# mohammadmarghzari/monte-carlo-portfolio

Hardware: AMD Instinct MI355X
Metric: simulated paths/sec (16 assets x 252 steps) + VaR abs-err vs NumPy ref (higher is better)
Workload: dtype f32; 1 GPU; configs[1]: 16 synthetic assets, 1,000,000 paths per GPU, 252 steps, fp32, full pass = paths + moments + exact VaR/CVaR; n_assets=16, n_steps=252, parallelism=path-sharded x1, math=exact

## Files before the change

### monte_carlo_portfolio_amd/csrc/mcp_api.cpp

```cpp
#include <hip/hip_runtime.h>
#include <dlfcn.h>

#include <algorithm>
#include <cmath>
#include <cstdarg>
#include <cstdio>
#include <cstdlib>
#include <cstring>
#include <mutex>
#include <new>
#include <string>
#include <vector>

#include "../../include/mcport.h"
#include "mcp_device.h"
#include "mcp_paths.h"
#include "mcp_stats_kernels.h"

#ifndef MCP_EXP_LEAN
#define MCP_EXP_LEAN 1
#endif

namespace {

thread_local std::string g_err;

int fail(int code, const char* fmt, ...) {
  char buf[512];
  va_list ap;
  va_start(ap, fmt);
  vsnprintf(buf, sizeof buf, fmt, ap);
  va_end(ap);
  g_err = buf;
  return code;
}

#define HIP_TRY(expr)                                                                       \
  do {                                                                                      \
    hipError_t e_ = (expr);                                                                 \
    if (e_ != hipSuccess) return fail(MCP_E_HIP, "%s: %s", #expr, hipGetErrorString(e_)); \
  } while (0)

constexpr int KT_WIDE = 8;
constexpr int K_PAD = 512;
using mcp::SWEEP_MIN_K;

int env_sweep_mt() {
  static const int v = [] { const char* e = getenv("MCP_SWEEP_MT"); return e ? atoi(e) : 0; }();
  return v;
}
bool uses_sweep(int K) { return K >= SWEEP_MIN_K && env_sweep_mt() >= 0; }
// ... 992 lines not shown
                              (unsigned long long*)ln.d_hist, ln.stream));
  fill_hz(s.hz, rq, ln);
  s.mdd = rq.dd ? ln.d_mdd : nullptr;
  s.mdd_stride = rq.dd ? ln.mdd_stride : 0;
  s.bt = boot_block(rq, ln);
  s.st = student_block(rq);
  if (rq.garch) s.gv = garch_block(rq.gv, N);
  if (rq.cash) s.cf.flows = ln.d_flows;
  if (rq.overlay) s.ov = overlay_block(rq, ln, N);
  if (rq.rebalanced) { s.period = rq.reb->period; s.cost = (float)rq.reb->cost; }
  if (rq.src == SRC_FHS) s.fh = filt_block(rq, ln, N);
  mcp::PathKernel k = {};
  k.logc = prm->compounding == MCP_COMPOUND_LOG;
  k.fh = rq.src == SRC_FHS;
  k.boot = rq.src == SRC_BOOT || k.fh;
  k.blds = k.fh ? mcp::filt_fits_lds((uint64_t)rq.filt->n_rows, nb) : k.boot && mcp::boot_fits_lds((uint64_t)rq.boot->n_rows, nb);
  k.stt = rq.src == SRC_T;
  if (ln.attr) {
    static const mcp_garch none = {0.0, 0.0, 1.0, 0};
    k.family = mcp::FAM_AT;
    k.stt = k.gv = true;
    a.partials = nullptr;
    a.hist = nullptr;
    if (!rq.garch) s.gv = garch_block(&none, N);
    s.at = attr_block(ln, N);
  } else {
    k.family = rq.overlay ? mcp::FAM_OV : rq.cash ? mcp::FAM_CF : rq.rebalanced ? mcp::FAM_REB : rq.dd ? mcp::FAM_DD : rq.hz ? mcp::FAM_HZ : mcp::FAM_PLAIN;
    k.dd = rq.overlay && rq.dd;
    k.gv = rq.garch;
    k.kt8 = K > 1;
    k.native = (prm->flags & MCP_FLAG_NATIVE_MATH) != 0;
    k.fold = (prm->flags & MCP_FLAG_FOLD) != 0;
    k.uhi = MCP_EXP_LEAN && plain && !rq.anti && !k.kt8 && !k.native && !k.fold && nb <= mcp::LEAN_MAX_NB && mcp::lean_range(a.path_begin, a.n_paths);
    if (rq.anti) {
      static const mcp_garch none = {0.0, 0.0, 1.0, 0};
      k.anti = true;
      if (k.stt || k.gv) {
        k.stt = k.gv = true;
        if (!rq.garch) s.gv = garch_block(&none, N);
      }
    }
  }
  const hipError_t e = k_launch[nb - 1](k, s, ln.stream);
  if (e != hipSuccess) return fail(MCP_E_HIP, "path kernel launch (family %d): %s", k.family, hipGetErrorString(e));
  return MCP_OK;
}

static Launch make_launch(const float* d_packed, const double* d_pivot, uint64_t seed, uint64_t path_begin, uint64_t n_paths,
                          float* d_terminal, uint64_t stride, void* d_partials, void* d_hist, void* stream) {
  Launch ln;
  ln.d_packed = d_packed;
  ln.d_pivot = d_pivot;
  ln.seed = seed;
  ln.path_begin = path_begin;
  ln.n_paths = n_paths;
  ln.d_terminal = d_terminal;
  ln.stride = stride;
  ln.d_partials = d_partials;
  ln.d_hist = d_hist;
  ln.stream = (hipStream_t)stream;
  return ln;
}

static int launch_checked(const mcp_params* prm, const Request& rq, const Launch& ln) {
  if (int rc = check_request(prm, rq, ln.n_paths, &ln)) return rc;
  return launch_paths_impl(prm, rq, ln);
// ... 1109 lines not shown
```

### monte_carlo_portfolio_amd/csrc/mcp_paths.h

```cpp
#pragma once
#include <hip/hip_runtime.h>
#include <stdint.h>

#include <type_traits>

#include "../../include/mcport.h"
#include "mcp_device.h"
#include "mcp_stats_kernels.h"

#ifndef MCP_MIN_WAVES
#define MCP_MIN_WAVES 6
#endif
#ifndef MCP_MIN_WAVES_BIG
#define MCP_MIN_WAVES_BIG 1
#endif
#ifndef MCP_MIN_WAVES_REB
#define MCP_MIN_WAVES_REB 5
#endif
#ifndef MCP_MIN_WAVES_REB8
#define MCP_MIN_WAVES_REB8 4
#endif
#ifndef MCP_MIN_WAVES_CF8
#define MCP_MIN_WAVES_CF8 5
#endif
#ifndef MCP_MIN_WAVES_OV
#define MCP_MIN_WAVES_OV 4
#endif
#ifndef MCP_MIN_WAVES_OV8
#define MCP_MIN_WAVES_OV8 4
#endif
#ifndef MCP_MIN_WAVES_AT
#define MCP_MIN_WAVES_AT 5
#endif
#ifndef MCP_MIN_WAVES_ANTI
#define MCP_MIN_WAVES_ANTI 5
#endif
#ifndef MCP_EXP_VKEYS
#define MCP_EXP_VKEYS 1
#endif
#ifndef MCP_EXP_BOOT_SWIZZLE
#define MCP_EXP_BOOT_SWIZZLE 1
#endif
#ifndef MCP_EXP_LDSPAR
#define MCP_EXP_LDSPAR 1
#endif

namespace mcp {

typedef float f32x2 __attribute__((ext_vector_type(2)));

#ifdef MCP_DIAG_CLOCK
extern __device__ unsigned long long mcp_diag_stamps[2 * 8192];
#endif

template <class A>
__device__ __forceinline__ const __attribute__((address_space(4))) A* kernarg() {
  typedef const __attribute__((address_space(4))) A* cst_p;
  cst_p k = (cst_p)__builtin_amdgcn_kernarg_segment_ptr();
  asm volatile("" : "+s"(k));
  return k;
}
#define MCP_HAS_MEMBER(m)                                                 \
  template <class A, class = void> struct has_##m : std::false_type {}; \
  template <class A> struct has_##m<A, std::void_t<decltype(A::m)>> : std::true_type {};
MCP_HAS_MEMBER(hz) MCP_HAS_MEMBER(mdd) MCP_HAS_MEMBER(bt) MCP_HAS_MEMBER(st) MCP_HAS_MEMBER(gv) MCP_HAS_MEMBER(cf)
MCP_HAS_MEMBER(ov) MCP_HAS_MEMBER(at) MCP_HAS_MEMBER(period) MCP_HAS_MEMBER(pr)
MCP_HAS_MEMBER(fh) MCP_HAS_MEMBER(p_hi)
#undef MCP_HAS_MEMBER

struct PathArgs {
  const float* __restrict__ packed;
  float* __restrict__ terminal;
  const float4* __restrict__ tables;
  const double* __restrict__ pivot;
  MomentPartial* __restrict__ partials;
  unsigned long long* __restrict__ hist;
  uint64_t slots;
  double v0d;
  double inv_v0d;
  int32_t v0_pow2;
  uint64_t seed, path_begin, n_paths, stride;
  int32_t n_steps, n_portfolios, k_begin, compounding;
  int32_t k_count;
  float v0;
  uint32_t fold_offset;
};

struct PathArgsLean : PathArgs {
  uint32_t p_hi;
  uint32_t pad;
};
template <class A>
__device__ __forceinline__ uint32_t uniform_hi(const A& a) {
  if constexpr (has_p_hi<A>::value) return a.p_hi;
  else return 0u;
}

struct PathArgsDD : PathArgs {
  float* __restrict__ mdd;
  uint64_t mdd_stride;
};

struct PathArgsHZ : PathArgs {
  float* __restrict__ hz;
  uint64_t hz_stride;
  int32_t n_horizons;
  int32_t steps[MCP_MAX_HORIZONS];
};

struct BootArgs {
  const float4* __restrict__ rows;
  uint64_t thr;
  uint32_t n_rows;
  uint32_t pad;
};
struct PathArgsBT : PathArgs { BootArgs bt; };
struct PathArgsBTHZ : PathArgsHZ { BootArgs bt; };
template <class A>
__device__ __forceinline__ BootArgs boot_args(const A& a) {
  if constexpr (has_bt<A>::value) return a.bt;
  else return BootArgs{};
}
struct PathArgsRB : PathArgsHZ {
  BootArgs bt;
  int32_t period;
  float cost;
};
struct StudentArgs {
// ... 127 lines not shown
}

struct PathLaunchArgs {
  PathArgsHZ hz;
  float* mdd;
  uint64_t mdd_stride;
  BootArgs bt;
  StudentArgs st;
  GarchArgs gv;
  CashArgs cf;
  OverlayArgs ov;
  AttrArgs at;
  int32_t period;
  float cost;
  PairArgs pr;
  FiltArgs fh;
};
template <class A>
inline A make_args(const PathLaunchArgs& s) {
  A x;
  if constexpr (has_hz<A>::value) static_cast<PathArgsHZ&>(x) = s.hz;
  else static_cast<PathArgs&>(x) = s.hz;
  if constexpr (has_mdd<A>::value) { x.mdd = s.mdd; x.mdd_stride = s.mdd_stride; }
  if constexpr (has_bt<A>::value) x.bt = s.bt;
  if constexpr (has_st<A>::value) x.st = s.st;
  if constexpr (has_gv<A>::value) x.gv = s.gv;
  if constexpr (has_cf<A>::value) x.cf = s.cf;
  if constexpr (has_ov<A>::value) x.ov = s.ov;
  if constexpr (has_at<A>::value) x.at = s.at;
  if constexpr (has_period<A>::value) { x.period = s.period; x.cost = s.cost; }
  if constexpr (has_pr<A>::value) x.pr = s.pr;
  if constexpr (has_fh<A>::value) x.fh = s.fh;
  if constexpr (has_p_hi<A>::value) { x.p_hi = (uint32_t)(s.hz.path_begin >> 32); x.pad = 0u; }
  return x;
}

__host__ __device__ constexpr bool boot_fits_lds(uint64_t n_rows, int nb) { return n_rows * (uint64_t)nb <= (uint64_t)ICDF_LDS_ENTRIES; }
__host__ __device__ constexpr bool filt_fits_lds(uint64_t n_rows, int nb) {
  return n_rows * (uint64_t)nb + (n_rows + 3) / 4 <= (uint64_t)ICDF_LDS_ENTRIES;
}
template <int NB>
struct BootSwizzle {
  static constexpr int G = (NB & -NB) > 16 ? 16 : (NB & -NB);
  static constexpr int SHIFT = G == 16 ? 0 : G == 8 ? 1 : G == 4 ? 2 : G == 2 ? 3 : 4;
  static constexpr uint32_t MASK = (uint32_t)G - 1u;
  __device__ static __forceinline__ uint32_t of(uint32_t j) { return MCP_EXP_BOOT_SWIZZLE ? (j >> SHIFT) & MASK : 0u; }
};

__device__ __forceinline__ double wave_sum(double v) {
#pragma unroll
  for (int o = 32; o > 0; o >>= 1) v += __shfl_xor(v, o, 64);
  return v;
}
__device__ __forceinline__ double wave_min(double v) {
#pragma unroll
  for (int o = 32; o > 0; o >>= 1) v = fmin(v, __shfl_xor(v, o, 64));
  return v;
}
__device__ __forceinline__ double wave_max(double v) {
#pragma unroll
  for (int o = 32; o > 0; o >>= 1) v = fmax(v, __shfl_xor(v, o, 64));
  return v;
}

__device__ __forceinline__ float wave_minf(float v) {
#pragma unroll
  for (int o = 32; o > 0; o >>= 1) v = fminf(v, __shfl_xor(v, o, 64));
  return v;
}
__device__ __forceinline__ float wave_maxf(float v) {
#pragma unroll
  for (int o = 32; o > 0; o >>= 1) v = fmaxf(v, __shfl_xor(v, o, 64));
  return v;
}

__device__ __forceinline__ void lds_hist_add(uint32_t* h, uint32_t digit, bool active) {
  unsigned long long todo = __ballot(active);
  const int lane = threadIdx.x & 63;
#pragma unroll 1
  for (int it = 0; it < 4 && todo; it++) {
    const int leader = __ffsll((long long)todo) - 1;
    const uint32_t d0 = (uint32_t)__builtin_amdgcn_readlane((int)digit, leader);
    const bool same = active && digit == d0;
    const unsigned long long m = __ballot(same);
    if (lane == leader) atomicAdd(&h[d0], (uint32_t)__popcll(m));
    todo &= ~m;
    active = active && !same;
  }
  if (active) atomicAdd(&h[digit], 1u);
}

__device__ __forceinline__ double terminal_to_x(float term, double v0, int compounding) {
  return compounding == MCP_COMPOUND_LOG ? expm1((double)term) : (double)term / v0 - 1.0;
}

constexpr int PATH_BLOCK = 256;

struct PathFlagsOff {
  static constexpr bool NATIVE = false, FOLD = false, LOGC = false, DD = false, HZ = false, BOOT = false, BLDS = false, REB = false,
                        STT = false, CF = false, OV = false, GV = false, AT = false, ANTI = false, FH = false, UHI = false;
};

enum BoundsKind { BK_PATHS, BK_REB, BK_CF, BK_OV, BK_AT, BK_ANTI };
constexpr int min_waves(BoundsKind kind, int NB, int KT, int PPT) {
  if (kind == BK_ANTI) return (NB <= 4 && PPT == 1 && KT == 1) ? MCP_MIN_WAVES_ANTI : 1;
  if (NB <= 4 && PPT == 1 && KT == 1)
    return kind == BK_REB ? MCP_MIN_WAVES_REB : kind == BK_OV ? MCP_MIN_WAVES_OV : kind == BK_AT ? MCP_MIN_WAVES_AT : MCP_MIN_WAVES;
  if (NB <= 4 && PPT == 1 && kind != BK_PATHS && kind != BK_AT)
    return kind == BK_REB ? MCP_MIN_WAVES_REB8 : kind == BK_CF ? MCP_MIN_WAVES_CF8 : MCP_MIN_WAVES_OV8;
  return (KT == 1 && PPT == 1) ? MCP_MIN_WAVES_BIG : 1;
}
#define MCP_BOUNDS(kind) __launch_bounds__(PATH_BLOCK, min_waves(kind, NB, KT, PPT))

template <int NB, int KT, int PPT, bool NATIVE_, bool FOLD_ = false, bool LOGC_ = false>
__global__ void MCP_BOUNDS(BK_PATHS) mc_paths_kernel(const PathArgs a) {
  struct F : PathFlagsOff { enum : bool { NATIVE = NATIVE_, FOLD = FOLD_, LOGC = LOGC_ }; };
#include "mcp_paths_body.inc"
}

template <int NB, bool LOGC_>
__global__ void __launch_bounds__(PATH_BLOCK, min_waves(BK_PATHS, NB, 1, 1)) mc_paths_lean_kernel(const PathArgsLean a) {
  constexpr int KT = 1, PPT = 1;
  struct F : PathFlagsOff { enum : bool { LOGC = LOGC_, UHI = true }; };
#include "mcp_paths_body.inc"
}

template <int NB, int KT, int PPT, bool LOGC_>
__global__ void MCP_BOUNDS(BK_PATHS) mc_paths_dd_kernel(const PathArgsDD a) {
  struct F : PathFlagsOff { enum : bool { DD = true, LOGC = LOGC_ }; };
#include "mcp_paths_body.inc"
}

template <int NB, int KT, int PPT, bool LOGC_>
__global__ void MCP_BOUNDS(BK_PATHS) mc_paths_hz_kernel(const PathArgsHZ a) {
  struct F : PathFlagsOff { enum : bool { HZ = true, LOGC = LOGC_ }; };
#include "mcp_paths_body.inc"
}

template <int NB, int KT, int PPT, bool LOGC_, bool BLDS_>
__global__ void MCP_BOUNDS(BK_PATHS) mc_paths_boot_kernel(const PathArgsBT a) {
  struct F : PathFlagsOff { enum : bool { BOOT = true, LOGC = LOGC_, BLDS = BLDS_ }; };
#include "mcp_paths_body.inc"
}

template <int NB, int KT, int PPT, bool LOGC_, bool BLDS_>
__global__ void MCP_BOUNDS(BK_PATHS) mc_paths_boot_hz_kernel(const PathArgsBTHZ a) {
  struct F : PathFlagsOff { enum : bool { HZ = true, BOOT = true, LOGC = LOGC_, BLDS = BLDS_ }; };
#include "mcp_paths_body.inc"
}
template <int NB, int KT, int PPT, bool BOOT_, bool BLDS_>
__global__ void MCP_BOUNDS(BK_REB) mc_paths_reb_kernel(const PathArgsRB a) {
  struct F : PathFlagsOff { enum : bool { REB = true, BOOT = BOOT_, BLDS = BLDS_ }; };
#include "mcp_paths_body.inc"
}

template <int NB, int KT, int PPT>
__global__ void MCP_BOUNDS(BK_PATHS) mc_paths_t_kernel(const PathArgsT a) {
  struct F : PathFlagsOff { enum : bool { STT = true }; };
#include "mcp_paths_body.inc"
// ... 65 lines not shown
```

### monte_carlo_portfolio_amd/csrc/mcp_paths_body.inc

```
  constexpr bool NATIVE = F::NATIVE, FOLD = F::FOLD, LOGC = F::LOGC, DD = F::DD, HZ = F::HZ, BOOT = F::BOOT, BLDS = F::BLDS, REB = F::REB,
                 STT = F::STT, CF = F::CF, OV = F::OV, GV = F::GV, AT = F::AT, ANTI = F::ANTI, FH = F::FH, UHI = F::UHI;
  static_assert(!UHI || (KT == 1 && PPT == 1 && !(NATIVE || FOLD || DD || HZ || BOOT || REB || STT || CF || OV || GV || AT || ANTI || FH)),
                "uniform high counter word: the plain Gaussian walk of one portfolio only");
  static_assert(!FH || (BOOT && HZ && !(LOGC || REB || CF || STT || GV || OV || AT || DD)), "filtered rows: the bootstrap's segmented walk only");
  constexpr int N4 = 4 * NB;
  constexpr int EM = ANTI ? 2 * PPT : PPT;
  static_assert(!ANTI || !(NATIVE || FOLD || BOOT || REB || CF || OV || AT || FH), "antithetic pairs: the lean Gaussian and GARCH walks only");
  typedef const __attribute__((address_space(4))) float* cfloat_p;
  cfloat_p mu = (cfloat_p)a.packed;
  cfloat_p Lp = mu + N4;
  cfloat_p Wk = mu + N4 + N4 * (N4 / 2 + 1) + (size_t)a.k_begin * N4;
  const int kt = min(KT, a.n_portfolios - a.k_begin);
  __shared__ float4 s_tab[ICDF_LDS_ENTRIES];
  if constexpr (!NATIVE && !BOOT) {
    for (int i = threadIdx.x; i < ICDF_ENTRIES; i += PATH_BLOCK) s_tab[ICDF_PAD + i] = a.tables[i];
  }
  BootArgs bt{};
  if constexpr (BOOT) bt = boot_args(a);
  if constexpr (BOOT && BLDS) {
    for (uint32_t i = threadIdx.x; i < bt.n_rows * (uint32_t)NB; i += PATH_BLOCK) {
      const uint32_t j = i / NB, q = i % NB;
      s_tab[j * NB + (q ^ BootSwizzle<NB>::of(j))] = bt.rows[i];
    }
  }
  const float* fshock = nullptr;
  if constexpr (FH) fshock = filt_args(a)->shock;
  if constexpr (FH && BLDS) {
    for (uint32_t i = threadIdx.x; i < (bt.n_rows + 3u) / 4u; i += PATH_BLOCK) s_tab[bt.n_rows * (uint32_t)NB + i] = ((const float4*)fshock)[i];
  }
  constexpr bool LDS_MU = MCP_EXP_LDSPAR >= 1 && !NATIVE && !FOLD && !BOOT;
  constexpr bool LDS_W = MCP_EXP_LDSPAR >= 2 && !NATIVE && !FOLD && !BOOT && KT == 1;
  float* const s_par0 = (float*)&s_tab[0];
  if constexpr (LDS_MU) {
    if (threadIdx.x < N4) { s_par0[threadIdx.x] = mu[threadIdx.x]; if (LDS_W) s_par0[N4 + threadIdx.x] = Wk[threadIdx.x]; }
// ... 11 lines not shown
  }
  if (threadIdx.x < PATH_BLOCK / 64) s_cnt[threadIdx.x] = 0ull;
  if constexpr (AT) {
    double* const s_at = attr_wave_slots<N4>();
    for (int i = threadIdx.x; i < (PATH_BLOCK / 64) * attr_record_len(N4); i += PATH_BLOCK) s_at[i] = 0.0;
  }
  if constexpr (ANTI) {
    if (threadIdx.x < (PATH_BLOCK / 64) * KT) pair_wave_slots<KT>()[threadIdx.x] = 0.0;
  }
  __syncthreads();
  const IcdfConsts kc = icdf_consts<UHI>();
  PhiloxKeys ks = philox_keys((uint32_t)a.seed, (uint32_t)(a.seed >> 32));
#if MCP_EXP_VKEYS
#pragma unroll
  for (int r = 0; r < 10; r++) { asm volatile("" : "+v"(ks.k0[r])); asm volatile("" : "+v"(ks.k1[r])); }
#endif
  typedef const __attribute__((address_space(3))) float* lfloat_p;
  PhiloxUniformKeys sk{};
  uint32_t uhi = 0u;
  lfloat_p par_lds = nullptr;
  if constexpr (UHI) {
    sk = philox_uniform_keys((uint32_t)a.seed, (uint32_t)(a.seed >> 32));
    uhi = uniform_hi(a);
    par_lds = (lfloat_p)s_par0;
  }
  const int T = a.n_steps;
  constexpr bool logc = LOGC;

  const uint64_t tile = (uint64_t)PATH_BLOCK * PPT;
  const uint64_t n_tiles = (a.n_paths + tile - 1) / tile;
#ifdef MCP_DIAG_CLOCK
  const unsigned long long diag_t0 = __builtin_amdgcn_s_memtime(), diag_r0 = __builtin_amdgcn_s_memrealtime();
#endif
  for (uint64_t tl = blockIdx.x; tl < n_tiles; tl += gridDim.x) {
    uint64_t p[PPT];
    bool live[PPT];
    uint32_t plo[PPT], phi[PPT];
    float V[EM][KT];
    float Pk[EM][KT], Qk[EM][KT];
    uint32_t jrow[PPT];
    f32x2 Bs[PPT][N4 / 2];
    float Ps[PPT][N4];
    float gh[PPT];
    f32x2 At[PPT][N4 / 2];
#pragma unroll
    for (int e = 0; e < PPT; e++) {
      p[e] = tl * tile + (uint64_t)e * PATH_BLOCK + threadIdx.x;
      live[e] = p[e] < a.n_paths;
      const uint64_t g = a.path_begin + p[e];
      plo[e] = (uint32_t)g; phi[e] = (uint32_t)(g >> 32);
#pragma unroll
      for (int k = 0; k < KT; k++) V[e][k] = logc ? 0.0f : a.v0;
      if constexpr (BOOT) jrow[e] = 0u;
      if constexpr (GV) gh[e] = garch_args(a)->h0;
      if constexpr (FH) gh[e] = filt_args(a)->h0;
      if constexpr (REB) {
#pragma unroll
        for (int m = 0; m < N4 / 2; m++) Bs[e][m] = f32x2{0.0f, 0.0f};
      }
      if constexpr (AT) {
#pragma unroll
        for (int m = 0; m < N4 / 2; m++) At[e][m] = f32x2{0.0f, 0.0f};
      }
      if constexpr (DD) {
#pragma unroll
        for (int k = 0; k < KT; k++) { Pk[e][k] = -__builtin_inff(); Qk[e][k] = logc ? 0.0f : 1.0f; }
      }
      if constexpr (OV) {
        typedef const __attribute__((address_space(4))) float* cspot_p;
        const cspot_p sp = (cspot_p)kernarg<PathArgsOV>()->ov.spot;
#pragma unroll
        for (int i = 0; i < N4; i++) Ps[e][i] = sp[i];
      }
      if constexpr (ANTI) {
#pragma unroll
        for (int k = 0; k < KT; k++) {
          V[PPT + e][k] = V[e][k];
          if constexpr (DD) { Pk[PPT + e][k] = Pk[e][k]; Qk[PPT + e][k] = Qk[e][k]; }
        }
      }
    }

    if constexpr (REB) {
      int nd;
      {
// ... 68 lines not shown
          for (int e = 0; e < PPT; e++)
#pragma unroll
            for (int m = 0; m < N4 / 2; m++) Bs[e][m] = f32x2{0.0f, 0.0f};
          const int per = cs->period;
          nd = per < T - t ? t + per : T;
        }
      }
    } else if constexpr (HZ) {
      typedef const __attribute__((address_space(4))) PathArgsHZ* chz_p;
      chz_p hk = (chz_p)__builtin_amdgcn_kernarg_segment_ptr();
      const int n_seg = hk->n_horizons + 1;
      int t = 0;
      for (int seg = 0; seg < n_seg; seg++) {
        const int t_end = seg < n_seg - 1 ? hk->steps[seg] : T;
        for (; t < t_end; t++) {
#include "mcp_paths_step.inc"
        }
        if (seg < n_seg - 1) {
          const auto hs = kernarg<PathArgsHZ>();
          float* const row = hs->hz + (size_t)(seg * a.n_portfolios + a.k_begin) * hs->hz_stride;
#pragma unroll
          for (int e = 0; e < PPT; e++)
            if (live[e]) {
#pragma unroll
              for (int k = 0; k < KT; k++)
                if (k < kt) {
                  if constexpr (ANTI) *(float2*)&row[(size_t)k * hs->hz_stride + 2 * p[e]] = make_float2(V[e][k], V[PPT + e][k]);
                  else row[(size_t)k * hs->hz_stride + p[e]] = V[e][k];
                }
            }
        }
      }
    } else {
      for (int t = 0; t < T; t++) {
#include "mcp_paths_step.inc"
      }
    }

    if constexpr (AT) {
      const auto ak = &kernarg<PathArgsAT>()->at;
      asm volatile("" : "+s"(kargs));
      const double e_c = kargs->pivot[a.k_begin], e_var = ak->var[a.k_begin], e_v0d = kargs->v0d;
      int tid = threadIdx.x;
      asm volatile("" : "+v"(tid));
      const int lane = tid & 63, wv = tid >> 6;
      double* const slot = attr_wave_slots<N4>() + wv * attr_record_len(N4);
      double dv[PPT];
      bool tail[PPT];
      double cn = 0.0, ct = 0.0, s1 = 0.0;
#pragma unroll
      for (int e = 0; e < PPT; e++) {
        const double x = terminal_to_x(V[e][0], e_v0d, MCP_COMPOUND_SIMPLE);
        tail[e] = live[e] && x <= e_var;
        dv[e] = live[e] ? x - e_c : 0.0;
        cn += live[e] ? 1.0 : 0.0;
        ct += tail[e] ? 1.0 : 0.0;
        s1 += dv[e];
      }
      cn = wave_sum(cn); ct = wave_sum(ct); s1 = wave_sum(s1);
      if (lane == 0) { slot[0] += cn; slot[1] += ct; slot[2] += s1; }
#pragma unroll
      for (int i = 0; i < N4; i++) {
        double sa = 0.0, st = 0.0, sx = 0.0;
#pragma unroll
        for (int e = 0; e < PPT; e++) {
          const double ai = live[e] ? (double)((i & 1) ? At[e][i / 2].y : At[e][i / 2].x) : 0.0;
          sa += ai;
// ... 14 lines not shown
            for (int e = 0; e < PPT; e++)
              if (live[e]) cb[((size_t)a.k_begin * n_live + i) * cs + p[e]] = (i & 1) ? At[e][i / 2].y : At[e][i / 2].x;
          }
      }
    } else {
#pragma unroll
    for (int e = 0; e < PPT; e++) {
      if (live[e]) {
#pragma unroll
        for (int k = 0; k < KT; k++)
          if (k < kt) {
            if constexpr (ANTI) *(float2*)&a.terminal[(size_t)(a.k_begin + k) * a.stride + 2 * p[e]] = make_float2(V[e][k], V[PPT + e][k]);
            else a.terminal[(size_t)(a.k_begin + k) * a.stride + p[e]] = V[e][k];
          }
        if constexpr (DD && OV) {
          const auto dk = kernarg<PathArgsOV>();
#pragma unroll
          for (int k = 0; k < KT; k++)
            if (k < kt) dk->mdd[(size_t)(a.k_begin + k) * dk->mdd_stride + p[e]] = Qk[e][k];
        } else if constexpr (DD) {
          const auto dk = kernarg<PathArgsDD>();
#pragma unroll
          for (int k = 0; k < KT; k++)
            if (k < kt) {
              if constexpr (ANTI) *(float2*)&dk->mdd[(size_t)(a.k_begin + k) * dk->mdd_stride + 2 * p[e]] = make_float2(Qk[e][k], Qk[PPT + e][k]);
              else dk->mdd[(size_t)(a.k_begin + k) * dk->mdd_stride + p[e]] = Qk[e][k];
            }
        }
      }
    }
    }

    asm volatile("" : "+s"(kargs));
    if (kargs->partials != nullptr) {
      const double* __restrict__ e_pivot = kargs->pivot;
      unsigned long long* __restrict__ e_hist = kargs->hist;
      const double e_v0d = kargs->v0d;
      int tid = threadIdx.x;
      asm volatile("" : "+v"(tid));
      const int lane = tid & 63, wv = tid >> 6;
      unsigned long long cnt = 0;
#pragma unroll
      for (int e = 0; e < PPT; e++) cnt += (unsigned long long)((EM / PPT) * __popcll(__ballot(live[e])));
      if (lane == 0) s_cnt[wv] += cnt;
#pragma unroll 1
      for (int k = 0; k < kt; k++) {
        const double c = e_pivot ? e_pivot[a.k_begin + k] : 0.0;
        double d1 = 0.0, d2 = 0.0;
        float mn = __builtin_inff(), mx = -__builtin_inff();
        double dm[EM];
#pragma unroll
        for (int e = 0; e < EM; e++) {
          float v = V[e][0];
#pragma unroll
          for (int kk = 1; kk < KT; kk++) v = (kk == k) ? V[e][kk] : v;
          if constexpr (ANTI) dm[e] = 0.0;
          if (live[e % PPT]) {
            const double d = terminal_to_x(v, e_v0d, logc ? MCP_COMPOUND_LOG : MCP_COMPOUND_SIMPLE) - c;
            d1 += d;
            d2 = __builtin_fma(d, d, d2);
            mn = fminf(mn, v);
            mx = fmaxf(mx, v);
            if constexpr (ANTI) dm[e] = d;
          }
          if (e_hist) lds_hist_add(s_hist, float_to_key(v) >> 21, live[e % PPT]);
        }
        d1 = wave_sum(d1); d2 = wave_sum(d2); mn = wave_minf(mn); mx = wave_maxf(mx);
        if (lane == 0) {
          s_mom[wv][k][0] += d1; s_mom[wv][k][1] += d2;
          s_ext[wv][k][0] = fminf(s_ext[wv][k][0], mn); s_ext[wv][k][1] = fmaxf(s_ext[wv][k][1], mx);
        }
        if constexpr (ANTI) {
          double cr = 0.0;
#pragma unroll
          for (int e = 0; e < PPT; e++) cr = __builtin_fma(dm[e], dm[PPT + e], cr);
          cr = wave_sum(cr);
          if (lane == 0) pair_wave_slots<KT>()[wv * KT + k] += cr;
        }
        if (e_hist) {
          __syncthreads();
          unsigned long long* out = e_hist + (size_t)(a.k_begin + k) * 2 * MCP_SELECT_BINS;
          for (int i = tid; i < MCP_SELECT_BINS; i += PATH_BLOCK) {
            const uint32_t h = s_hist[i];
            if (h) { atomicAdd(&out[i], (unsigned long long)h); s_hist[i] = 0u; }
          }
          __syncthreads();
        }
      }
    }
  }

#ifdef MCP_DIAG_CLOCK
  if (threadIdx.x == 0 && blockIdx.x < 8192) {
    mcp_diag_stamps[2 * blockIdx.x] = __builtin_amdgcn_s_memtime() - diag_t0;
    mcp_diag_stamps[2 * blockIdx.x + 1] = __builtin_amdgcn_s_memrealtime() - diag_r0;
  }
#endif
  asm volatile("" : "+s"(kargs));
  if (kargs->partials != nullptr) {
    __syncthreads();
    if ((int)threadIdx.x < kt) {
      const int k = threadIdx.x;
      MomentPartial o;
      o.s1 = (s_mom[0][k][0] + s_mom[1][k][0]) + (s_mom[2][k][0] + s_mom[3][k][0]);
      o.s2 = (s_mom[0][k][1] + s_mom[1][k][1]) + (s_mom[2][k][1] + s_mom[3][k][1]);
      o.vmin = fminf(fminf(s_ext[0][k][0], s_ext[1][k][0]), fminf(s_ext[2][k][0], s_ext[3][k][0]));
      o.vmax = fmaxf(fmaxf(s_ext[0][k][1], s_ext[1][k][1]), fmaxf(s_ext[2][k][1], s_ext[3][k][1]));
      o.n = (s_cnt[0] + s_cnt[1]) + (s_cnt[2] + s_cnt[3]);
      kargs->partials[(size_t)(a.k_begin + k) * kargs->slots + blockIdx.x] = o;
      if constexpr (ANTI) {
        const double* const s_cr = pair_wave_slots<KT>();
        pair_cross(a)[(size_t)(a.k_begin + k) * gridDim.x + blockIdx.x] = (s_cr[k] + s_cr[KT + k]) + (s_cr[2 * KT + k] + s_cr[3 * KT + k]);
      }
    }
  }
  if constexpr (AT) {
    __syncthreads();
    const auto ak = &kernarg<PathArgsAT>()->at;
    const double* const s_at = attr_wave_slots<N4>();
    constexpr int RL = attr_record_len(N4);
    if ((int)threadIdx.x < RL) {
      const int j = threadIdx.x;
      ak->partials[((size_t)a.k_begin * gridDim.x + blockIdx.x) * RL + j] = (s_at[j] + s_at[RL + j]) + (s_at[2 * RL + j] + s_at[3 * RL + j]);
    }
  }
```

### monte_carlo_portfolio_amd/csrc/mcp_paths_inst.hip

```cpp
#include <cstdlib>

#include "mcp_paths.h"
#include "mcp_stats_kernels.h"

#ifndef MCP_NB
#error "compile with -DMCP_NB=<1..16>"
#endif

#define MCP_CAT_(a, b) a##b
#define MCP_CAT(a, b) MCP_CAT_(a, b)

namespace mcp {

static size_t lds_pad() {
  static const size_t pad = [] { const char* e = getenv("MCP_PATHS_LDS_PAD"); return e ? (size_t)atol(e) : (size_t)0; }();
  return pad;
}

template <int KT, class A>
static hipError_t run(void (*kernel)(A), const PathLaunchArgs& s, hipStream_t stream) {
  A x = make_args<A>(s);
  const int grid = path_grid(x.n_paths);
  for (x.k_begin = 0; x.k_begin < x.n_portfolios; x.k_begin += KT) {
    kernel<<<grid, PATH_BLOCK, lds_pad(), stream>>>(x);
    const hipError_t e = hipGetLastError();
    if (e != hipSuccess) return e;
  }
  return hipSuccess;
}
#define MCP_ROW(cond, ...) \
  if (cond) return run<KT>(__VA_ARGS__, s, stream)

template <int KT>
static hipError_t ladder(const PathKernel& k, const PathLaunchArgs& s, hipStream_t stream) {
  constexpr int NB = MCP_NB;
  const bool lg = k.logc;
  const bool gauss = !k.boot && !k.stt && !k.gv;
  const bool t = k.stt && !k.gv && !k.boot, g = k.gv && !k.boot;
  const bool bl = k.boot && k.blds && !k.stt && !k.gv && !k.fh, bg = k.boot && !k.blds && !k.stt && !k.gv && !k.fh;
  if (k.fh) {
    const bool ok = (k.family == FAM_PLAIN || k.family == FAM_HZ) && k.boot && !k.stt && !k.gv && !k.native && !k.anti && !lg;
    MCP_ROW(ok && k.blds, mc_paths_fhs_kernel<NB, KT, 1, true>);
    MCP_ROW(ok && !k.blds, mc_paths_fhs_kernel<NB, KT, 1, false>);
    return hipErrorInvalidValue;
  }
  if (k.anti) {
    const bool lean = gauss && !k.native, gw = k.stt && k.gv && !k.boot && !k.native && !lg;
    switch (k.family) {
      case FAM_PLAIN:
        MCP_ROW(lean && lg, mc_paths_anti_kernel<NB, KT, 1, true, PathArgsA>);
        MCP_ROW(lean && !lg, mc_paths_anti_kernel<NB, KT, 1, false, PathArgsA>);
        MCP_ROW(gw, mc_paths_anti_kernel<NB, KT, 1, false, PathArgsGA>);
        break;
      case FAM_DD:
        MCP_ROW(lean && lg, mc_paths_anti_kernel<NB, KT, 1, true, PathArgsADD>);
        MCP_ROW(lean && !lg, mc_paths_anti_kernel<NB, KT, 1, false, PathArgsADD>);
        MCP_ROW(gw, mc_paths_anti_kernel<NB, KT, 1, false, PathArgsGADD>);
        break;
      case FAM_HZ:
// ... 40 lines not shown
      MCP_ROW(gauss && !lg, mc_paths_reb_kernel<NB, KT, 1, false, false>);
      MCP_ROW(bl && !lg, mc_paths_reb_kernel<NB, KT, 1, true, true>);
      MCP_ROW(bg && !lg, mc_paths_reb_kernel<NB, KT, 1, true, false>);
      break;
    case FAM_CF:
      MCP_ROW(gauss && !lg, mc_paths_cf_kernel<NB, KT, 1, false, false, false>);
      MCP_ROW(t && !lg, mc_paths_cf_kernel<NB, KT, 1, false, false, true>);
      MCP_ROW(bl && !lg, mc_paths_cf_kernel<NB, KT, 1, true, true, false>);
      MCP_ROW(bg && !lg, mc_paths_cf_kernel<NB, KT, 1, true, false, false>);
      break;
    case FAM_OV:
      MCP_ROW(gauss && !lg && !k.dd, mc_paths_ov_kernel<NB, KT, 1, false, false>);
      MCP_ROW(gauss && !lg && k.dd, mc_paths_ov_kernel<NB, KT, 1, false, true>);
      MCP_ROW(t && !lg && !k.dd, mc_paths_ov_kernel<NB, KT, 1, true, false>);
      MCP_ROW(t && !lg && k.dd, mc_paths_ov_kernel<NB, KT, 1, true, true>);
      break;
  }
  return hipErrorInvalidValue;
}

hipError_t MCP_CAT(launch_paths_nb, MCP_NB)(const PathKernel& k, const PathLaunchArgs& s, hipStream_t stream) {
  constexpr int NB = MCP_NB, KT = 1;
  if (k.anti && (k.fold || k.family == FAM_AT)) return hipErrorInvalidValue;
  if (k.fh && (k.fold || k.family == FAM_AT)) return hipErrorInvalidValue;
  if (k.fold) {
    const bool ok = k.family == FAM_PLAIN && !k.boot && !k.stt && !k.gv && !k.native && !k.kt8;
    MCP_ROW(ok && k.logc, mc_paths_kernel<NB, 1, 1, false, true, true>);
    MCP_ROW(ok && !k.logc, mc_paths_kernel<NB, 1, 1, false, true, false>);
    return hipErrorInvalidValue;
  }
  if (k.uhi) {
    if constexpr (NB <= LEAN_MAX_NB) {
      const bool ok = k.family == FAM_PLAIN && !k.boot && !k.stt && !k.gv && !k.native && !k.kt8 && !k.anti && !k.fh;
      MCP_ROW(ok && k.logc, mc_paths_lean_kernel<NB, true>);
      MCP_ROW(ok && !k.logc, mc_paths_lean_kernel<NB, false>);
    }
    return hipErrorInvalidValue;
  }
  if (k.family == FAM_AT) {
    MCP_ROW(!k.kt8 && !k.native && !k.logc && !k.boot, mc_paths_attr_kernel<NB, 1, 1>);
    return hipErrorInvalidValue;
  }
  return k.kt8 ? ladder<8>(k, s, stream) : ladder<1>(k, s, stream);
}
#undef MCP_ROW

}
```

### monte_carlo_portfolio_amd/csrc/mcp_route.h

```cpp
#pragma once
#include <stdint.h>

namespace mcp {

inline bool lean_range(uint64_t path_begin, uint64_t n_paths) {
  if (n_paths == 0) return false;
  const uint64_t last = path_begin + (n_paths - 1);
  return last >= path_begin && (path_begin >> 32) == (last >> 32);
}

}
```

### monte_carlo_portfolio_amd/csrc/mcp_stats_kernels.h

```cpp
#pragma once
#include <hip/hip_runtime.h>
#include <stdint.h>

#include "../../include/mcport.h"
#include "mcp_route.h"

namespace mcp {

struct SelectState {
  uint32_t prefix;
  uint32_t pad;
  uint64_t rank;
};

struct Quantile {
  double x_lo, x_hi, var;
  double level2;
  uint64_t n_tail;
  uint64_t pad;
};

struct MomentPartial {
  double s1, s2;
  float vmin, vmax;
  unsigned long long n;
};
static_assert(sizeof(MomentPartial) == 32, "MomentPartial is 32 bytes");

constexpr int PATH_GRID_CAP = 8192;
constexpr int SWEEP_MIN_K = 17;
constexpr int SWEEP_TILE_PATHS = 64;

__host__ __device__ inline int path_grid(uint64_t n) {
  uint64_t tiles = (n + 255) / 256;
  if (tiles < 1) tiles = 1;
  return (int)(tiles < (uint64_t)PATH_GRID_CAP ? tiles : (uint64_t)PATH_GRID_CAP);
}
__host__ __device__ inline uint64_t moment_slots(bool sweep, uint64_t n) {
  return sweep ? (n + SWEEP_TILE_PATHS - 1) / SWEEP_TILE_PATHS + (n == 0) : (uint64_t)path_grid(n);
}

__host__ __device__ inline int stream_slots(int K) {
  const int s = 16384 / (K < 1 ? 1 : K);
  return s > 2048 ? 2048 : (s < 1 ? 1 : s);
}

struct PathArgs;
struct PathLaunchArgs;

constexpr int LEAN_MAX_NB = 4;
enum PathFamily { FAM_PLAIN, FAM_DD, FAM_HZ, FAM_REB, FAM_CF, FAM_OV, FAM_AT };
struct PathKernel {
  int family;
  bool logc, boot, blds, stt, dd, gv, kt8, native, fold, anti, fh, uhi;
};

typedef hipError_t (*launch_paths_fn)(const PathKernel& k, const PathLaunchArgs& args, hipStream_t stream);
#define MCP_DECL_NB(n) hipError_t launch_paths_nb##n(const PathKernel& k, const PathLaunchArgs& args, hipStream_t stream);
MCP_DECL_NB(1) MCP_DECL_NB(2) MCP_DECL_NB(3) MCP_DECL_NB(4) MCP_DECL_NB(5) MCP_DECL_NB(6) MCP_DECL_NB(7) MCP_DECL_NB(8)
MCP_DECL_NB(9) MCP_DECL_NB(10) MCP_DECL_NB(11) MCP_DECL_NB(12) MCP_DECL_NB(13) MCP_DECL_NB(14) MCP_DECL_NB(15) MCP_DECL_NB(16)
#undef MCP_DECL_NB

hipError_t launch_sweep_shared(int nb, int mt, bool native, const PathArgs& args, hipStream_t stream);
hipError_t launch_sweep_shared_p0(int nb, int mt, bool native, const PathArgs& args, hipStream_t stream);
hipError_t launch_sweep_shared_p1(int nb, int mt, bool native, const PathArgs& args, hipStream_t stream);
hipError_t launch_sweep_shared_p2(int nb, int mt, bool native, const PathArgs& args, hipStream_t stream);
hipError_t launch_sweep_shared_p3(int nb, int mt, bool native, const PathArgs& args, hipStream_t stream);
hipError_t launch_sweep_paths(int nb, int mt, bool native, const PathArgs& args, hipStream_t stream);
hipError_t launch_normals(const uint32_t* x, uint64_t n, const float4* table, float* z, hipStream_t s);

hipError_t launch_pass0(const mcp_params& prm, int K, const float* terminal, uint64_t stride, uint64_t n, const double* pivot,
                        uint64_t slots, MomentPartial* partials, unsigned long long* hist, hipStream_t s);
hipError_t launch_scan(const mcp_params& prm, int K, int pass, uint64_t n, uint64_t rank_lo, uint64_t rank_hi, uint64_t slots,
                       const MomentPartial* partials, const double* below, const double* pivot, unsigned long long* hist,
                       SelectState* state, mcp_record* record, hipStream_t s);
hipError_t launch_hist(const mcp_params& prm, int K, int pass, const float* terminal, uint64_t stride, uint64_t n,
                       const SelectState* state, const double* pivot, double* below, unsigned long long* hist, hipStream_t s);
hipError_t launch_final(const mcp_params& prm, int K, uint64_t n, double gamma, uint64_t rank_lo, uint64_t rank_hi,
                        const double* below, unsigned long long* hist, const SelectState* state, mcp_record* record,
                        Quantile* quant, mcp_stats* stats_or_null, hipStream_t s);
hipError_t launch_stats(const mcp_params& prm, int K, int world, const mcp_record* gathered, const Quantile* quant,
                        mcp_stats* out, hipStream_t s);
hipError_t launch_zero(void* p, size_t bytes, hipStream_t s);
hipError_t launch_count_rows(const float* values, uint64_t stride, uint64_t n, int rows, bool has_target, float target,
                             unsigned long long* counts, hipStream_t s);
hipError_t launch_sum_u64(unsigned long long* const* bufs, int nsrc, size_t words, hipStream_t s);
hipError_t launch_attr_merge(const double* partials, int K, int blocks, int len, double* out, hipStream_t s);
// ... 7 lines not shown
```

Before: 447.9 million paths/s.

## Split lean path walk into time segments to fill tail waves

Adds a segmented variant of the lean path kernel. Each launch covers a whole number of resident-block waves of (tile, time-segment) units, and the path value is carried between segments through the terminal buffer. A host-side cost model picks the segment count from occupancy and the tile count, to cut the idle tail of the last partial wave. The trade is extra launches, a global read and write of path state at each segment boundary, and a reliance on the RNG being addressable by step so the walk can resume mid-path.

```diff
diff --git a/monte_carlo_portfolio_amd/csrc/mcp_api.cpp b/monte_carlo_portfolio_amd/csrc/mcp_api.cpp
--- a/monte_carlo_portfolio_amd/csrc/mcp_api.cpp
+++ b/monte_carlo_portfolio_amd/csrc/mcp_api.cpp
@@ -17,6 +17,9 @@
 #include "mcp_paths.h"
 #include "mcp_stats_kernels.h"
 
+#ifndef MCP_EXP_SEGMENTS
+#define MCP_EXP_SEGMENTS 1
+#endif
 #ifndef MCP_EXP_LEAN
 #define MCP_EXP_LEAN 1
 #endif
@@ -1075,6 +1078,13 @@
     k.native = (prm->flags & MCP_FLAG_NATIVE_MATH) != 0;
     k.fold = (prm->flags & MCP_FLAG_FOLD) != 0;
     k.uhi = MCP_EXP_LEAN && plain && !rq.anti && !k.kt8 && !k.native && !k.fold && nb <= mcp::LEAN_MAX_NB && mcp::lean_range(a.path_begin, a.n_paths);
+    if (k.uhi) {
+      const char* const ks = getenv("MCP_TIME_SEGMENTS");
+      const char* const cs = getenv("MCP_SEGMENT_CAP");
+      const long kf = ks ? atol(ks) : 0, cf = cs ? atol(cs) : 0;
+      k.seg_forced = !MCP_EXP_SEGMENTS ? 1 : kf < 0 ? 0 : kf > prm->n_steps ? prm->n_steps : (int32_t)kf;
+      k.seg_cap = cf > 0 && cf <= (long)mcp::SEG_GRID_CAP ? (uint32_t)cf : 0u;
+    }
     if (rq.anti) {
       static const mcp_garch none = {0.0, 0.0, 1.0, 0};
       k.anti = true;
diff --git a/monte_carlo_portfolio_amd/csrc/mcp_paths.h b/monte_carlo_portfolio_amd/csrc/mcp_paths.h
--- a/monte_carlo_portfolio_amd/csrc/mcp_paths.h
+++ b/monte_carlo_portfolio_amd/csrc/mcp_paths.h
@@ -6,6 +6,7 @@
 
 #include "../../include/mcport.h"
 #include "mcp_device.h"
+#include "mcp_route.h"
 #include "mcp_stats_kernels.h"
 
 #ifndef MCP_MIN_WAVES
@@ -65,7 +66,7 @@
   template <class A> struct has_##m<A, std::void_t<decltype(A::m)>> : std::true_type {};
 MCP_HAS_MEMBER(hz) MCP_HAS_MEMBER(mdd) MCP_HAS_MEMBER(bt) MCP_HAS_MEMBER(st) MCP_HAS_MEMBER(gv) MCP_HAS_MEMBER(cf)
 MCP_HAS_MEMBER(ov) MCP_HAS_MEMBER(at) MCP_HAS_MEMBER(period) MCP_HAS_MEMBER(pr)
-MCP_HAS_MEMBER(fh) MCP_HAS_MEMBER(p_hi)
+MCP_HAS_MEMBER(fh) MCP_HAS_MEMBER(p_hi) MCP_HAS_MEMBER(first_unit)
 #undef MCP_HAS_MEMBER
 
 struct PathArgs {
@@ -94,6 +95,21 @@
 __device__ __forceinline__ uint32_t uniform_hi(const A& a) {
   if constexpr (has_p_hi<A>::value) return a.p_hi;
   else return 0u;
+}
+
+struct PathArgsSeg : PathArgsLean {
+  uint32_t first_unit;
+  int32_t n_seg;
+};
+template <class A>
+__device__ __forceinline__ uint32_t seg_first_unit(const A& a) {
+  if constexpr (has_first_unit<A>::value) return a.first_unit;
+  else return 0u;
+}
+template <class A>
+__device__ __forceinline__ int32_t seg_count(const A& a) {
+  if constexpr (has_first_unit<A>::value) return a.n_seg;
+  else return 1;
 }
 
 struct PathArgsDD : PathArgs {
@@ -287,6 +303,7 @@
   if constexpr (has_pr<A>::value) x.pr = s.pr;
   if constexpr (has_fh<A>::value) x.fh = s.fh;
   if constexpr (has_p_hi<A>::value) { x.p_hi = (uint32_t)(s.hz.path_begin >> 32); x.pad = 0u; }
+  if constexpr (has_first_unit<A>::value) { x.first_unit = 0u; x.n_seg = 1; }
   return x;
 }
 
@@ -350,10 +367,11 @@
 }
 
 constexpr int PATH_BLOCK = 256;
+static_assert(SEG_GRID_CAP == (uint64_t)PATH_GRID_CAP, "segment_plan keeps grid-strided launches whole");
 
 struct PathFlagsOff {
   static constexpr bool NATIVE = false, FOLD = false, LOGC = false, DD = false, HZ = false, BOOT = false, BLDS = false, REB = false,
-                        STT = false, CF = false, OV = false, GV = false, AT = false, ANTI = false, FH = false, UHI = false;
+                        STT = false, CF = false, OV = false, GV = false, AT = false, ANTI = false, FH = false, UHI = false, SEG = false;
 };
 
 enum BoundsKind { BK_PATHS, BK_REB, BK_CF, BK_OV, BK_AT, BK_ANTI };
@@ -380,6 +398,13 @@
 #include "mcp_paths_body.inc"
 }
 
+template <int NB, bool LOGC_>
+__global__ void __launch_bounds__(PATH_BLOCK, min_waves(BK_PATHS, NB, 1, 1)) mc_paths_lean_seg_kernel(const PathArgsSeg a) {
+  constexpr int KT = 1, PPT = 1;
+  struct F : PathFlagsOff { enum : bool { LOGC = LOGC_, UHI = true, SEG = true }; };
+#include "mcp_paths_body.inc"
+}
+
 template <int NB, int KT, int PPT, bool LOGC_>
 __global__ void MCP_BOUNDS(BK_PATHS) mc_paths_dd_kernel(const PathArgsDD a) {
   struct F : PathFlagsOff { enum : bool { DD = true, LOGC = LOGC_ }; };
diff --git a/monte_carlo_portfolio_amd/csrc/mcp_paths_body.inc b/monte_carlo_portfolio_amd/csrc/mcp_paths_body.inc
--- a/monte_carlo_portfolio_amd/csrc/mcp_paths_body.inc
+++ b/monte_carlo_portfolio_amd/csrc/mcp_paths_body.inc
@@ -1,5 +1,6 @@
   constexpr bool NATIVE = F::NATIVE, FOLD = F::FOLD, LOGC = F::LOGC, DD = F::DD, HZ = F::HZ, BOOT = F::BOOT, BLDS = F::BLDS, REB = F::REB,
-                 STT = F::STT, CF = F::CF, OV = F::OV, GV = F::GV, AT = F::AT, ANTI = F::ANTI, FH = F::FH, UHI = F::UHI;
+                 STT = F::STT, CF = F::CF, OV = F::OV, GV = F::GV, AT = F::AT, ANTI = F::ANTI, FH = F::FH, UHI = F::UHI, SEG = F::SEG;
+  static_assert(!SEG || UHI, "time segments: the lean kernel only");
   static_assert(!UHI || (KT == 1 && PPT == 1 && !(NATIVE || FOLD || DD || HZ || BOOT || REB || STT || CF || OV || GV || AT || ANTI || FH)),
                 "uniform high counter word: the plain Gaussian walk of one portfolio only");
   static_assert(!FH || (BOOT && HZ && !(LOGC || REB || CF || STT || GV || OV || AT || DD)), "filtered rows: the bootstrap's segmented walk only");
@@ -77,7 +78,19 @@
 #ifdef MCP_DIAG_CLOCK
   const unsigned long long diag_t0 = __builtin_amdgcn_s_memtime(), diag_r0 = __builtin_amdgcn_s_memrealtime();
 #endif
-  for (uint64_t tl = blockIdx.x; tl < n_tiles; tl += gridDim.x) {
+  uint64_t seg_tile = 0;
+  int seg_t0 = 0, seg_t1 = T;
+  bool seg_first = true, seg_last = true;
+  if constexpr (SEG) {
+    const uint32_t u = seg_first_unit(a) + blockIdx.x, nt = (uint32_t)n_tiles;
+    const int sg = (int)(u / nt), n_seg = seg_count(a);
+    seg_tile = sg < n_seg ? (uint64_t)(u - (uint32_t)sg * nt) : n_tiles;
+    seg_t0 = segment_begin(sg, T, n_seg);
+    seg_t1 = segment_begin(sg + 1, T, n_seg);
+    seg_first = sg == 0;
+    seg_last = sg == n_seg - 1;
+  }
+  for (uint64_t tl = SEG ? seg_tile : (uint64_t)blockIdx.x; tl < n_tiles; tl += SEG ? n_tiles : (uint64_t)gridDim.x) {
     uint64_t p[PPT];
     bool live[PPT];
     uint32_t plo[PPT], phi[PPT];
@@ -96,6 +109,9 @@
       plo[e] = (uint32_t)g; phi[e] = (uint32_t)(g >> 32);
 #pragma unroll
       for (int k = 0; k < KT; k++) V[e][k] = logc ? 0.0f : a.v0;
+      if constexpr (SEG) {
+        if (!seg_first && live[e]) V[e][0] = a.terminal[(size_t)a.k_begin * a.stride + p[e]];
+      }
       if constexpr (BOOT) jrow[e] = 0u;
       if constexpr (GV) gh[e] = garch_args(a)->h0;
       if constexpr (FH) gh[e] = filt_args(a)->h0;
@@ -230,7 +246,7 @@
         }
       }
     } else {
-      for (int t = 0; t < T; t++) {
+      for (int t = SEG ? seg_t0 : 0; t < (SEG ? seg_t1 : T); t++) {
 #include "mcp_paths_step.inc"
       }
     }
@@ -311,7 +327,7 @@
     }
 
     asm volatile("" : "+s"(kargs));
-    if (kargs->partials != nullptr) {
+    if ((!SEG || seg_last) && kargs->partials != nullptr) {
       const double* __restrict__ e_pivot = kargs->pivot;
       unsigned long long* __restrict__ e_hist = kargs->hist;
       const double e_v0d = kargs->v0d;
@@ -376,7 +392,7 @@
   }
 #endif
   asm volatile("" : "+s"(kargs));
-  if (kargs->partials != nullptr) {
+  if ((!SEG || (seg_last && seg_tile < n_tiles)) && kargs->partials != nullptr) {
     __syncthreads();
     if ((int)threadIdx.x < kt) {
       const int k = threadIdx.x;
@@ -386,7 +402,7 @@
       o.vmin = fminf(fminf(s_ext[0][k][0], s_ext[1][k][0]), fminf(s_ext[2][k][0], s_ext[3][k][0]));
       o.vmax = fmaxf(fmaxf(s_ext[0][k][1], s_ext[1][k][1]), fmaxf(s_ext[2][k][1], s_ext[3][k][1]));
       o.n = (s_cnt[0] + s_cnt[1]) + (s_cnt[2] + s_cnt[3]);
-      kargs->partials[(size_t)(a.k_begin + k) * kargs->slots + blockIdx.x] = o;
+      kargs->partials[(size_t)(a.k_begin + k) * kargs->slots + (SEG ? seg_tile : (uint64_t)blockIdx.x)] = o;
       if constexpr (ANTI) {
         const double* const s_cr = pair_wave_slots<KT>();
         pair_cross(a)[(size_t)(a.k_begin + k) * gridDim.x + blockIdx.x] = (s_cr[k] + s_cr[KT + k]) + (s_cr[2 * KT + k] + s_cr[3 * KT + k]);
diff --git a/monte_carlo_portfolio_amd/csrc/mcp_paths_inst.hip b/monte_carlo_portfolio_amd/csrc/mcp_paths_inst.hip
--- a/monte_carlo_portfolio_amd/csrc/mcp_paths_inst.hip
+++ b/monte_carlo_portfolio_amd/csrc/mcp_paths_inst.hip
@@ -1,3 +1,4 @@
+#include <atomic>
 #include <cstdlib>
 
 #include "mcp_paths.h"
@@ -25,6 +26,50 @@
     kernel<<<grid, PATH_BLOCK, lds_pad(), stream>>>(x);
     const hipError_t e = hipGetLastError();
     if (e != hipSuccess) return e;
+  }
+  return hipSuccess;
+}
+
+template <bool LOGC>
+static hipError_t resident_blocks(uint32_t* cap) {
+  void (*const kernel)(PathArgsSeg) = mc_paths_lean_seg_kernel<MCP_NB, LOGC>;
+  constexpr int MAX_DEV = 64;
+  static std::atomic<uint32_t> cached[MAX_DEV];
+  int dev = 0;
+  hipError_t e = hipGetDevice(&dev);
+  if (e != hipSuccess) return e;
+  if (dev >= 0 && dev < MAX_DEV && (*cap = cached[dev].load(std::memory_order_relaxed)) != 0u) return hipSuccess;
+  int per_cu = 0, cus = 0;
+  if ((e = hipOccupancyMaxActiveBlocksPerMultiprocessor(&per_cu, kernel, PATH_BLOCK, lds_pad())) != hipSuccess) return e;
+  if ((e = hipDeviceGetAttribute(&cus, hipDeviceAttributeMultiprocessorCount, dev)) != hipSuccess) return e;
+  *cap = (uint32_t)(per_cu > 0 ? per_cu : 0) * (uint32_t)(cus > 0 ? cus : 0);
+  if (dev >= 0 && dev < MAX_DEV) cached[dev].store(*cap, std::memory_order_relaxed);
+  return hipSuccess;
+}
+
+template <bool LOGC>
+static hipError_t run_lean(const PathKernel& k, const PathLaunchArgs& s, hipStream_t stream) {
+  void (*const whole)(PathArgsLean) = mc_paths_lean_kernel<MCP_NB, LOGC>;
+  void (*const seg)(PathArgsSeg) = mc_paths_lean_seg_kernel<MCP_NB, LOGC>;
+  const uint64_t n_tiles = (s.hz.n_paths + PATH_BLOCK - 1) / PATH_BLOCK;
+  uint32_t cap = k.seg_cap;
+  if (k.seg_forced != 1 && cap == 0u) {
+    const hipError_t e = resident_blocks<LOGC>(&cap);
+    if (e != hipSuccess) return e;
+  }
+  const SegmentPlan plan = segment_plan(n_tiles, s.hz.n_steps, cap, k.seg_forced);
+  if (plan.k == 1) return run<1>(whole, s, stream);
+  PathArgsSeg x = make_args<PathArgsSeg>(s);
+  x.n_seg = plan.k;
+  const uint64_t units = n_tiles * (uint64_t)plan.k;
+  for (x.k_begin = 0; x.k_begin < x.n_portfolios; x.k_begin++) {
+    for (uint64_t u = 0; u < units; u += plan.launch_units) {
+      x.first_unit = (uint32_t)u;
+      const uint64_t grid = units - u < plan.launch_units ? units - u : plan.launch_units;
+      seg<<<(unsigned)grid, PATH_BLOCK, lds_pad(), stream>>>(x);
+      const hipError_t e = hipGetLastError();
+      if (e != hipSuccess) return e;
+    }
   }
   return hipSuccess;
 }
@@ -131,8 +176,7 @@
   if (k.uhi) {
     if constexpr (NB <= LEAN_MAX_NB) {
       const bool ok = k.family == FAM_PLAIN && !k.boot && !k.stt && !k.gv && !k.native && !k.kt8 && !k.anti && !k.fh;
-      MCP_ROW(ok && k.logc, mc_paths_lean_kernel<NB, true>);
-      MCP_ROW(ok && !k.logc, mc_paths_lean_kernel<NB, false>);
+      if (ok) return k.logc ? run_lean<true>(k, s, stream) : run_lean<false>(k, s, stream);
     }
     return hipErrorInvalidValue;
   }
diff --git a/monte_carlo_portfolio_amd/csrc/mcp_route.h b/monte_carlo_portfolio_amd/csrc/mcp_route.h
--- a/monte_carlo_portfolio_amd/csrc/mcp_route.h
+++ b/monte_carlo_portfolio_amd/csrc/mcp_route.h
@@ -9,4 +9,48 @@
   return last >= path_begin && (path_begin >> 32) == (last >> 32);
 }
 
+constexpr int32_t segment_begin(int32_t s, int32_t n_steps, int32_t k) {
+  return s * (n_steps / k) + (s < n_steps % k ? s : n_steps % k);
 }
+
+constexpr double SEG_TAIL_LATENCY = 0.10;
+constexpr double SEG_C_UNIT = 0.0010;
+constexpr double SEG_C_BOUNDARY = 0.0013;
+constexpr int32_t SEG_MIN_STEPS = 16;
+constexpr double SEG_MIN_GAIN = 0.006;
+constexpr uint64_t SEG_GRID_CAP = 8192;
+
+struct SegmentPlan {
+  int32_t k;
+  uint32_t launch_units;
+};
+
+inline double segment_model(uint64_t n_tiles, uint64_t cap, int32_t k) {
+  const uint64_t units = n_tiles * (uint64_t)k;
+  const uint64_t per_launch = k == 1 ? units : cap * (n_tiles / cap);
+  const uint64_t launches = (units + per_launch - 1) / per_launch;
+  const uint64_t full = units / cap, rest = units % cap;
+  const double tail = rest == 0 ? 0.0 : SEG_TAIL_LATENCY + (1.0 - SEG_TAIL_LATENCY) * (double)rest / (double)cap;
+  return ((double)full + tail) / (double)k + (double)(full + (rest != 0)) * SEG_C_UNIT + (double)launches * SEG_C_BOUNDARY;
+}
+
+inline SegmentPlan segment_plan(uint64_t n_tiles, int32_t n_steps, uint64_t cap, int32_t k_forced) {
+  const SegmentPlan whole = {1, 0u};
+  if (cap == 0 || n_tiles < cap || n_tiles > SEG_GRID_CAP || n_steps < 2 || k_forced == 1 || k_forced < 0) return whole;
+  int32_t k = 1;
+  if (k_forced >= 2) {
+    k = k_forced < n_steps ? k_forced : n_steps;
+  } else {
+    const double t1 = segment_model(n_tiles, cap, 1);
+    double best = t1 * (1.0 - SEG_MIN_GAIN);
+    for (int32_t c = 2; c <= n_steps / SEG_MIN_STEPS; c++) {
+      const double t = segment_model(n_tiles, cap, c);
+      if (t < best) { best = t; k = c; }
+    }
+  }
+  if (k == 1 || n_tiles * (uint64_t)k > (1ull << 31)) return whole;
+  const SegmentPlan plan = {k, (uint32_t)(cap * (n_tiles / cap))};
+  return plan;
+}
+
+}
diff --git a/monte_carlo_portfolio_amd/csrc/mcp_stats_kernels.h b/monte_carlo_portfolio_amd/csrc/mcp_stats_kernels.h
--- a/monte_carlo_portfolio_amd/csrc/mcp_stats_kernels.h
+++ b/monte_carlo_portfolio_amd/csrc/mcp_stats_kernels.h
@@ -53,6 +53,8 @@
 struct PathKernel {
   int family;
   bool logc, boot, blds, stt, dd, gv, kt8, native, fold, anti, fh, uhi;
+  int32_t seg_forced;
+  uint32_t seg_cap;
 };
 
 typedef hipError_t (*launch_paths_fn)(const PathKernel& k, const PathLaunchArgs& args, hipStream_t stream);
```

After: 445.7 million paths/s. No clear change (-0.5%).
